# Chlumsky/msdfgen

Hardware: AMD Instinct MI355X
Metric: MSDF glyphs/sec (64x64, fp32) (higher is better)
Workload: dtype f64

## Files before the change

### msdfgen_amd/csrc/msdf_ec_fast.hpp

```cpp
#pragma once

#include "msdf_ec.hpp"

namespace msdfhip {

enum { EC_DEFER = 0x80 };

enum { EC_V_ERROR = 1,
       EC_V_CHECK = 2,
       EC_V_COND = 4,
       EC_V_HELD = 8 };
enum { EC_ORDER_EAGER = 0, EC_ORDER_LAZY = 1, EC_ORDER_LAZY_HELD = 2 };

MSDF_HD bool ecHasBasePass(const EcParams &p) { return p.distanceCheck == EC_DO_NOT_CHECK || (p.distanceCheck == EC_CHECK_AT_EDGE && p.mode != EC_MODE_EDGE_ONLY); }
MSDF_HD bool ecHasShapePass(const EcParams &p) { return p.distanceCheck == EC_ALWAYS_CHECK || p.distanceCheck == EC_CHECK_AT_EDGE; }
MSDF_HD bool ecLazyProtect(const EcParams &p) { return p.mode == EC_MODE_EDGE_PRIORITY && p.distanceCheck == EC_CHECK_AT_EDGE; }

struct FastCtx {
    double span;
    bool p1;
    bool pShape;
    bool basePass, shapePass;
    int order;
};

MSDF_HD int rangeTest2(const FastCtx &c, double at, double bt, double xt, float am, float bm, float xm) {
    const bool inversion = (am > .5f && bm > .5f && xm <= .5f) || (am < .5f && bm < .5f && xm >= .5f);
    const bool outside = medianf(am, bm, xm) != xm;
    const bool candBase = c.basePass && (inversion || (!c.p1 && outside));
    const bool candShape = c.shapePass && (inversion || (!c.pShape && outside));
    const bool candCond = c.order != EC_ORDER_EAGER && !inversion && outside;
    if (!(candBase || candShape || candCond))
        return 0;
    const double axSpan = (xt-at)*c.span, bxSpan = (bt-xt)*c.span;
    const int f = (xm >= am-axSpan && xm <= am+axSpan && xm >= bm-bxSpan && xm <= bm+bxSpan) ? 1 : 3;
    return (candBase ? f : 0)|(candShape ? f<<2 : 0)|(candCond && f == 3 ? 16 : 0);
}

MSDF_HD int judge(int flags) {
    const int cond = (flags&16) ? EC_V_COND : 0;
    if (flags&2)
        return EC_V_ERROR|cond;
    const int fs = (flags>>2)&3;
    if (fs&1)
        return ((fs&2) ? EC_V_ERROR : EC_V_CHECK)|cond;
    return cond;
}

MSDF_HD bool quadraticMayHaveRootInRange(double a, double b, double c) {
    if (a == 0 || fabs(b) > 1e12*fabs(a))
        return true;
    const double lo = .005, hi = .995;
    const double mag = fabs(a)+fabs(b)+fabs(c);
    const double eps = 1e-9*mag;
    const double flo = (a*lo+b)*lo+c, fhi = (a*hi+b)*hi+c;
    if (!(flo > eps && fhi > eps) && !(flo < -eps && fhi < -eps))
        return true;
    const double s = flo > 0 ? 1. : -1.;
    const double as = a*s, bs = b*s, cs = c*s;
    if (as <= 0)
        return false;
    if (!(-bs > 2*as*lo*(1-1e-9) && -bs < 2*as*hi*(1+1e-9)))
        return false;
    return !(4*as*cs-bs*bs > 1e-9*mag*mag);
}

MSDF_HD bool bernsteinMayHaveRoot(float dA, float dBC, float dD) {
    const float m = fmaxf(fmaxf(fabsf(dA), fabsf(dBC)), fabsf(dD));
    const float eps = 1e-5f*m;
    const float h = .5f*dBC;
    return !((dA > eps && h > eps && dD > eps) || (dA < -eps && h < -eps && dD < -eps));
}

MSDF_HD bool edgeBetweenTexelsChannelFast(const float *a, const float *b, int channel) {
    const double n = a[channel]-.5;
    const double d = a[channel]-b[channel];
    if (!((n > 0 && d > 0 && n < d) || (n < 0 && d < 0 && n > d)))
        return false;
    const double t = n/d;
    if (t > 0 && t < 1) {
        float c[3] = { mixf(a[0], b[0], t), mixf(a[1], b[1], t), mixf(a[2], b[2], t) };
        return medianf(c[0], c[1], c[2]) == c[channel];
    }
    return false;
}

MSDF_HD int edgeBetweenTexelsFast(const float *a, const float *b) {
    return 1*(int) edgeBetweenTexelsChannelFast(a, b, 0)+2*(int) edgeBetweenTexelsChannelFast(a, b, 1)+4*(int) edgeBetweenTexelsChannelFast(a, b, 2);
}

template <class Sink>
MSDF_HD int diagonalPairFast(const FastCtx &cx, float am, float dm, const float *a, const float *l, const float *q,
                             float dA, float dBC, float dD, float l0, float q0, float l1, float q1, Sink &sink) {
    const double qa = dD-dBC+dA, qb = dBC-dA-dA, qc = dA;
    if (!quadraticMayHaveRootInRange(qa, qb, qc))
        return 0;
    double t[2];
    const int solutions = solveQuadratic(t, qa, qb, qc);
    int verdict = 0;
    for (int i = 0; i < solutions; ++i) {
        if (t[i] > MSDF_ARTIFACT_T_EPSILON && t[i] < 1-MSDF_ARTIFACT_T_EPSILON) {
            const float xm = interpolatedMedianQuad(a, l, q, t[i]);
            int rangeFlags = rangeTest2(cx, 0, 1, t[i], am, dm, xm);
            const double tEx0 = -.5*l0/q0, tEx1 = -.5*l1/q1;
            if (tEx0 > 0 && tEx0 < 1) {
                double tEnd0 = 0, tEnd1 = 1;
                float em0 = am, em1 = dm;
                const float ex = interpolatedMedianQuad(a, l, q, tEx0);
                if (tEx0 > t[i])
                    tEnd1 = tEx0, em1 = ex;
                else
                    tEnd0 = tEx0, em0 = ex;
                rangeFlags |= rangeTest2(cx, tEnd0, tEnd1, t[i], em0, em1, xm);
            }
            if (tEx1 > 0 && tEx1 < 1) {
                double tEnd0 = 0, tEnd1 = 1;
                float em0 = am, em1 = dm;
                const float ex = interpolatedMedianQuad(a, l, q, tEx1);
                if (tEx1 > t[i])
                    tEnd1 = tEx1, em1 = ex;
                else
                    tEnd0 = tEx1, em0 = ex;
                rangeFlags |= rangeTest2(cx, tEnd0, tEnd1, t[i], em0, em1, xm);
            }
            const int v = judge(rangeFlags);
            verdict |= v;
            if (v&EC_V_CHECK) {
                const bool held = (verdict&EC_V_COND) != 0;
                if (held)
                    verdict |= EC_V_HELD;
                if (held == (cx.order == EC_ORDER_LAZY_HELD))
                    sink(t[i]);
            }
            if (verdict&EC_V_ERROR)
                return verdict;
        }
    }
    return verdict;
}

struct Neighbourhood {
    float v[3][3][3];
    float dev[3][3];
    unsigned valid;
};

MSDF_HD float ecTexelDeviation(const float *t) { return fabsf(medianf(t[0], t[1], t[2])-.5f); }

MSDF_HD void loadNeighbourhood(Neighbourhood &nb, const SdfView &sdf, int x, int yn) {
    nb.valid = 0;
    MSDF_UNROLL
    for (int dy = -1; dy <= 1; ++dy) {
        MSDF_UNROLL
        for (int dx = -1; dx <= 1; ++dx) {
            const int nx = x+dx, ny = yn+dy;
            const bool in = nx >= 0 && ny >= 0 && nx < sdf.w && ny < sdf.h;
            const float *t = sdf.native(in ? nx : x, in ? ny : yn);
            nb.v[dy+1][dx+1][0] = t[0], nb.v[dy+1][dx+1][1] = t[1], nb.v[dy+1][dx+1][2] = t[2];
            nb.dev[dy+1][dx+1] = ecTexelDeviation(t);
            if (in)
                nb.valid |= 1u<<((dy+1)*3+(dx+1));
        }
    }
}

template <class Emit>
MSDF_HD void texelProtectPairs(const Neighbourhood &nb, const EcParams &p, Emit &emit) {
    const float sdev = nb.dev[1][1];
    MSDF_UNROLL
    for (int dy = -1; dy <= 1; ++dy) {
        MSDF_UNROLL
        for (int dx = -1; dx <= 1; ++dx) {
            if (!dx && !dy)
                continue;
            if (!(nb.valid&(1u<<((dy+1)*3+(dx+1)))))
                continue;
            const float radius = dy == 0 ? p.radiusH : dx == 0 ? p.radiusV : p.radiusD;
            const float odev = nb.dev[dy+1][dx+1];
            const bool selfIsA = dy > 0 || (dy == 0 && dx > 0);
            const float sum = selfIsA ? sdev+odev : odev+sdev;
            if (sum < radius)
                emit((dy+1)*3+(dx+1));
        }
    }
}

MSDF_HD bool evaluateProtectPair(const float *self, const float *other, int m) {
    const int dy = m/3-1, dx = m%3-1;
    const bool selfIsA = dy > 0 || (dy == 0 && dx > 0);
    const int mask = selfIsA ? edgeBetweenTexelsFast(self, other) : edgeBetweenTexelsFast(other, self);
    return extremeChannelInMask(self, medianf(self[0], self[1], self[2]), mask);
}

MSDF_HD bool protectedByEdgesNb(const Neighbourhood &nb, const EcParams &p) {
    struct Items {
        unsigned char m[8];
        int n;
        MSDF_HD void operator()(int mm) { m[n++] = (unsigned char) mm; }
    } items;
    items.n = 0;
    texelProtectPairs(nb, p, items);
    for (int i = 0; i < items.n; ++i)
        if (evaluateProtectPair(nb.v[1][1], nb.v[items.m[i]/3][items.m[i]%3], items.m[i]))
            return true;
    return false;
}

MSDF_HD int ecNeighbourDx(int k) { return k < 4 ? (k == 0 ? -1 : k == 2 ? 1 : 0) : ((k&1) ? 1 : -1); }
MSDF_HD int ecNeighbourDy(int k) { return k < 4 ? (k == 1 ? -1 : k == 3 ? 1 : 0) : ((k&2) ? 1 : -1); }

template <class Emit>
MSDF_HD void texelCandidatePairs(const Neighbourhood &nb, Emit &emit) {
    const float *c = nb.v[1][1];
    const float cdev = nb.dev[1][1];
    MSDF_UNROLL
    for (int k = 0; k < 4; ++k) {
        const int dx = k == 0 ? -1 : k == 2 ? 1 : 0, dy = k == 1 ? -1 : k == 3 ? 1 : 0;
        if (!(nb.valid&(1u<<((dy+1)*3+(dx+1)))))
            continue;
        const float *b = nb.v[dy+1][dx+1];
        if (!(cdev >= nb.dev[dy+1][dx+1]))
            continue;
        MSDF_UNROLL
        for (int j = 0; j < 3; ++j) {
            const int i0 = j, i1 = j == 2 ? 0 : j+1;
            const float dA = c[i1]-c[i0], dB = b[i1]-b[i0];
            if ((dA > 0 && dB < 0) || (dA < 0 && dB > 0))
                emit(k, j);
        }
    }
    MSDF_UNROLL
    for (int k = 4; k < 8; ++k) {
        const int dx = (k&1) ? 1 : -1, dy = (k&2) ? 1 : -1;
        if (!(nb.valid&(1u<<((dy+1)*3+(dx+1)))))
            continue;
        const float *d = nb.v[dy+1][dx+1];
        if (!(cdev >= nb.dev[dy+1][dx+1]))
            continue;
        const float *b = nb.v[1][dx+1], *cc = nb.v[dy+1][1];
        MSDF_UNROLL
        for (int j = 0; j < 3; ++j) {
            const int i0 = j, i1 = j == 2 ? 0 : j+1;
            const float dA = c[i1]-c[i0], dBC = b[i1]-b[i0]+cc[i1]-cc[i0], dD = d[i1]-d[i0];
            if (dA == 0 && dBC == 0 && dD == 0)
                continue;
            if (bernsteinMayHaveRoot(dA, dBC, dD))
                emit(k, j);
        }
    }
}

MSDF_HD float pick3(const float *v, int i) { return i == 0 ? v[0] : i == 1 ? v[1] : v[2]; }

template <class Sink>
MSDF_HD int evaluatePair(const float *c, const float *n, const float *hb, const float *vc, const EcParams &p, bool p1, int flip, int k, int j, Sink &sink,
                         int order = EC_ORDER_EAGER) {
    FastCtx cx;
    cx.basePass = ecHasBasePass(p);
    cx.shapePass = ecHasShapePass(p);
    cx.order = order;
    cx.p1 = order != EC_ORDER_EAGER || p1;
    cx.pShape = (p.distanceCheck == EC_CHECK_AT_EDGE) ? true : cx.p1;
    const int dx = ecNeighbourDx(k), dy = ecNeighbourDy(k);
    const int i0 = j, i1 = j == 2 ? 0 : j+1;
    const float cm = medianf(c[0], c[1], c[2]), nm = medianf(n[0], n[1], n[2]);
    if (k < 4) {
        if (order == EC_ORDER_LAZY_HELD)
            return 0;
        cx.span = dy == 0 ? p.hSpan : p.vSpan;
        const float dA = pick3(c, i1)-pick3(c, i0), dB = pick3(n, i1)-pick3(n, i0);
        const double t = (double) dA/(dA-dB);
        if (t > MSDF_ARTIFACT_T_EPSILON && t < 1-MSDF_ARTIFACT_T_EPSILON) {
            const float xm = interpolatedMedianLin(c, n, t);
            const int v = judge(rangeTest2(cx, 0, 1, t, cm, nm, xm));
            if (v&EC_V_CHECK)
                sink(t, dx, flip ? -dy : dy);
            return v;
        }
        return 0;
    }
    cx.span = p.dSpan;
    const float *a = c, *b = hb, *cc = vc, *d = n;
    const float abc[3] = { a[0]-b[0]-cc[0], a[1]-b[1]-cc[1], a[2]-b[2]-cc[2] };
    const float l[3] = { -a[0]-abc[0], -a[1]-abc[1], -a[2]-abc[2] };
    const float q[3] = { d[0]+abc[0], d[1]+abc[1], d[2]+abc[2] };
    const float a3[3] = { a[0], a[1], a[2] };
    struct DirSink {
        Sink &sink;
        int dx, dy;
        MSDF_HD void operator()(double t) { sink(t, dx, dy); }
    } dirSink = { sink, dx, flip ? -dy : dy };
    const float dA = pick3(a, i1)-pick3(a, i0), dBC = pick3(b, i1)-pick3(b, i0)+pick3(cc, i1)-pick3(cc, i0), dD = pick3(d, i1)-pick3(d, i0);
    return diagonalPairFast(cx, cm, nm, a3, l, q, dA, dBC, dD, pick3(l, i0), pick3(q, i0), pick3(l, i1), pick3(q, i1), dirSink);
}

template <class Sink>
MSDF_HD int texelFindFast(const Neighbourhood &nb, const EcParams &p, bool p1, int flip, Sink &sink, int order = EC_ORDER_EAGER) {
    struct Items {
        unsigned char k[24], j[24];
        int n;
        MSDF_HD void operator()(int kk, int jj) { k[n] = (unsigned char) kk, j[n] = (unsigned char) jj; ++n; }
    } items;
    items.n = 0;
    texelCandidatePairs(nb, items);
    int verdict = 0;
    for (int i = 0; i < items.n; ++i) {
        const int k = items.k[i], dx = ecNeighbourDx(k), dy = ecNeighbourDy(k);
        verdict |= evaluatePair(nb.v[1][1], nb.v[dy+1][dx+1], nb.v[1][dx+1], nb.v[dy+1][1], p, p1, flip, k, items.j[i], sink, order);
    }
    return verdict;
}

MSDF_HD bool protectedByCornerList(const int *corners, int nCorners, int x, int ys) {
    for (int i = 0; i < nCorners; ++i) {
        const int l = corners[2*i], b = corners[2*i+1];
        if ((x == l || x == l+1) && (ys == b || ys == b+1))
            return true;
    }
    return false;
}

MSDF_HD bool ecNeedsProtection(int verdict) { return ((verdict&EC_V_COND) && !(verdict&EC_V_ERROR)) || (verdict&EC_V_HELD); }

template <class Sink>
MSDF_HD int ecTexelFast(const SdfView &sdf, const EcParams &p, const int *corners, int nCorners, int x, int yn, Sink &sink, bool allowLazy = true) {
    const int ys = sdf.flip ? sdf.h-1-yn : yn;
    Neighbourhood nb;
    loadNeighbourhood(nb, sdf, x, yn);
    int st = 0, verdict;
    if (allowLazy && ecLazyProtect(p)) {
        verdict = texelFindFast(nb, p, true, sdf.flip, sink, EC_ORDER_LAZY);
        if (ecNeedsProtection(verdict)) {
            if (!(protectedByCornerList(corners, nCorners, x, ys) || protectedByEdgesNb(nb, p)))
                verdict |= EC_V_ERROR;
            else if (verdict&EC_V_HELD)
                texelFindFast(nb, p, true, sdf.flip, sink, EC_ORDER_LAZY_HELD);
        }
    } else {
        if (p.mode == EC_MODE_EDGE_PRIORITY) {
            if (protectedByCornerList(corners, nCorners, x, ys) || protectedByEdgesNb(nb, p))
                st |= EC_PROTECTED;
        } else if (p.mode == EC_MODE_EDGE_ONLY)
            st |= EC_PROTECTED;
        verdict = texelFindFast(nb, p, (st&EC_PROTECTED) != 0, sdf.flip, sink);
    }
    if (ecHasBasePass(p) && p.distanceCheck == EC_CHECK_AT_EDGE)
        st |= EC_PROTECTED;
    if (verdict&EC_V_ERROR)
        st |= EC_ERROR;
    else if (verdict&EC_V_CHECK)
        st |= EC_DEFER;
    return st;
}

template <class Query>
MSDF_HD bool ecEvaluateCandidate(const SdfView &sdf, const EcParams &p, int x, int ys, double t, int dx, int dy, const Query &query) {
    const float *msd = sdf.shape(x, ys);
    const V2 tVector = t*mk(dx, dy);
    float oldMSD[3], newMSD[3];
    interpolate3(oldMSD, sdf, mk(x+.5, ys+.5)+tVector);
    const double aWeight = (1-fabs(tVector.x))*(1-fabs(tVector.y));
    const float aPSD = medianf(msd[0], msd[1], msd[2]);
    newMSD[0] = (float) (oldMSD[0]+aWeight*(aPSD-msd[0]));
    newMSD[1] = (float) (oldMSD[1]+aWeight*(aPSD-msd[1]));
    newMSD[2] = (float) (oldMSD[2]+aWeight*(aPSD-msd[2]));
    const float oldPSD = medianf(oldMSD[0], oldMSD[1], oldMSD[2]);
    const float newPSD = medianf(newMSD[0], newMSD[1], newMSD[2]);
    const V2 q = unproject(p.t, mk(x+.5, ys+.5))+mk(tVector.x*p.texelX, tVector.y*p.texelY);
    const float refPSD = mapDistance(p.t, query(q));
    return p.minImproveRatio*fabsf(newPSD-refPSD) < (double) fabsf(oldPSD-refPSD);
}

}
```

### msdfgen_amd/csrc/msdf_kernels.hpp

```cpp
#pragma once

#include <hip/hip_runtime.h>
#include "msdf_device.hpp"
#include "msdf_prep.hpp"
#include "msdf_ec.hpp"
#include "msdf_ec_fast.hpp"
#include "msdf_cull.hpp"
#include "msdf_scanline.hpp"
#include "msdf_shapeprep.hpp"
#include "msdf_frame.hpp"
#include "../../include/msdfgen_hip.h"

namespace msdfhip {

#ifndef MSDF_DISTANCE_WAVES_PER_SIMD
#define MSDF_DISTANCE_WAVES_PER_SIMD 4
#endif
constexpr int TILE = 8;
constexpr int WAVE = 64;
constexpr int REC_DOUBLES = sizeof(EdgeRec)/sizeof(double);

struct BatchView {
    int nGlyphs;
    const int32_t *glyphContourOffsets;
// ... 781 lines not shown
    mutable unsigned long long cached;
    int cacheCap;
#if defined(MSDF_PROFILE_QUERY)
    mutable unsigned long long prof[16];
#endif
    MSDF_HD int begin(int c) const { return coff[c]-coff[0]; }
    MSDF_HD int end(int c) const { return coff[c+1]-coff[0]; }
};
#if defined(MSDF_PROFILE_QUERY)
__device__ inline unsigned long long qNow() {
#if MSDF_PROFILE_QUERY >= 2
    asm volatile("s_waitcnt vmcnt(0) lgkmcnt(0)" ::: "memory");
#endif
    return __builtin_readcyclecounter();
}
__device__ inline void profAdd(const EdgesCooperative &edges, int i, unsigned long long dt) { edges.prof[i] += dt; }
__device__ inline unsigned long long profNow(const EdgesCooperative &) { return qNow(); }
__device__ unsigned long long gQueryDetail[16];
#endif

__device__ inline void selAddContour(Selector<2> &sel, const EdgeRec *rec, const EdgesCooperative &edges, int c, V2 o) {
    if (edges.slots) {
        if (c == 0) {
#if defined(MSDF_PROFILE_QUERY)
            const unsigned long long qa = qNow();
#endif
            for (int base = 0; base < edges.nE; base += WAVE) {
                const int i = base+edges.lane;
                if (i < edges.nE) {
                    Selector<2> mine;
                    selInit(mine);
                    const EdgeRegs r = loadEdgeRegs(rec+i, i);
                    selAddEdge(mine, r, i, o);
                    edges.slots[i] = mine.c[0];
                }
            }
            waveSync();
#if defined(MSDF_PROFILE_QUERY)
            const unsigned long long qb = qNow();
            edges.prof[0] += qb-qa;
#endif
            for (int cc = edges.lane; cc < edges.C; cc += WAVE) {
                PB acc;
                pbInit(acc);
                const int e = edges.end(cc);
                for (int i = edges.begin(cc); i < e; ++i) {
                    const PBSlot one = edges.slots[i];
                    pbMerge(acc, one);
                }
                edges.merged[cc] = acc;
            }
            waveSync();
#if defined(MSDF_PROFILE_QUERY)
            edges.prof[1] += qNow()-qb;
#endif
        }
        const PBSlot whole = edges.merged[c];
        pbMerge(sel.c[0], whole);
        return;
    }
    const bool cacheable = c < 64 && c < edges.cacheCap;
    if (cacheable && ((edges.cached>>c)&1ull)) {
        const PBSlot whole = edges.merged[c];
        pbMerge(sel.c[0], whole);
        return;
    }
    PB contour;
    pbInit(contour);
    const int e = edges.end(c);
    for (int base = edges.begin(c); base < e; base += WAVE) {
        Selector<2> mine;
        selInit(mine);
        const int i = base+edges.lane;
        if (i < e) {
            const EdgeRegs r = loadEdgeRegs(rec+i, i);
            selAddEdge(mine, r, i, o);
        }
        PB &m = mine.c[0];
        MSDF_UNROLL
        for (int off = 1; off < WAVE; off <<= 1) {
            PB other;
            other.td = __shfl_down(m.td, off), other.tdot = __shfl_down(m.tdot, off), other.perp = __shfl_down(m.perp, off);
            other.neg = __shfl_down(m.neg, off), other.pos = __shfl_down(m.pos, off);
            if (edges.lane+off < WAVE)
                pbMerge(m, other);
        }
        PB all;
        all.td = __shfl(m.td, 0), all.tdot = __shfl(m.tdot, 0), all.perp = __shfl(m.perp, 0), all.neg = __shfl(m.neg, 0), all.pos = __shfl(m.pos, 0);
        pbMerge(contour, all);
    }
    pbMerge(sel.c[0], contour);
    if (cacheable) {
        edges.merged[c] = contour;
        edges.cached |= 1ull<<c;
        waveSync();
    }
}

template <bool OVERLAP, class Wind = const int8_t *>
struct PsdfQueryCooperative {
    const EdgeRec *rec;
    const int32_t *coff;
    Wind windings;
    int C, lane;
    double *res;
    PBSlot *slots, *merged;
    int cacheCap = 0;
    __device__ double operator()(V2 q) const {
        double out[1];
        EdgesCooperative edges;
        edges.coff = coff, edges.lane = lane, edges.slots = slots, edges.merged = merged, edges.nE = coff[C]-coff[0], edges.C = C;
        edges.cached = 0, edges.cacheCap = slots ? 0 : cacheCap;
#if defined(MSDF_PROFILE_QUERY)
        for (int i = 0; i < 16; ++i)
            edges.prof[i] = 0;
        const unsigned long long qq0 = qNow();
#endif
        if (slots)
            waveSync();
        if (OVERLAP)
            shapeDistanceOverlap<2>(rec, edges, windings, C, q, res, 1, out);
        else
            shapeDistanceSimple<2>(rec, edges, C, q, out);
#if defined(MSDF_PROFILE_QUERY)
        if (lane == 0) {
            atomicAdd(&gQueryDetail[0], 1ull), atomicAdd(&gQueryDetail[1], qNow()-qq0);
            atomicAdd(&gQueryDetail[2], edges.prof[0]), atomicAdd(&gQueryDetail[3], edges.prof[1]), atomicAdd(&gQueryDetail[4], edges.prof[8]);
            atomicAdd(&gQueryDetail[5], edges.prof[9]), atomicAdd(&gQueryDetail[6], edges.prof[10]), atomicAdd(&gQueryDetail[7], edges.prof[11]);
            atomicAdd(&gQueryDetail[8], (unsigned long long) C), atomicAdd(&gQueryDetail[9], (unsigned long long) (slots ? 1 : 0));
        }
#endif
        return out[0];
    }
};

struct EcCandidate {
    unsigned texel;
    int dir;
    double t;
};
static_assert(sizeof(EcCandidate) == 16, "EcCandidate layout");

MSDF_HD size_t ecHeaderRecords(int nGlyphs) { return ((size_t) (nGlyphs+1)*sizeof(unsigned)+sizeof(EcCandidate)-1)/sizeof(EcCandidate); }
MSDF_HD unsigned ecSegment(size_t texelsPerGlyph) { return (unsigned) (texelsPerGlyph/8 > 64 ? (texelsPerGlyph/8+63)/64*64 : 64); }

struct CandidateSink {
    unsigned *header;
    EcCandidate *segment;
    unsigned seg, texel;
    int g;
    __device__ void operator()(double t, int dx, int dy) {
        const unsigned slot = atomicAdd(&header[1+g], 1u);
        if (slot < seg) {
            EcCandidate c;
            c.texel = texel, c.dir = (dx+1)|((dy+1)<<2), c.t = t;
            segment[slot] = c;
        } else
            header[0] = 1u;
    }
};

MSDF_HD size_t stencilIndex(size_t texel, int yn, int width, int height, int stencilYDown) {
    return stencilYDown ? texel+(size_t) (height-1-2*yn)*width : texel;
}

struct EcGlyphParams {
    double hSpan, vSpan, dSpan, texelX, texelY;
    float radiusH, radiusV, radiusD;
    int cornerBegin, nCorners;
    int pad;
};
static_assert(sizeof(EcGlyphParams) == 64, "EcGlyphParams layout");

__device__ __forceinline__ void ecParamsBody(EcGlyphParams *out, const BatchView &batch, const MsdfHipGlyph *glyphs, const MsdfHipConfig &cfg, unsigned *candidateHeader,
                                             int *corners, int *sizes, const int g, const int lane) {
    if (candidateHeader && lane == 0) {
        candidateHeader[1+g] = 0;
        if (g == 0)
            candidateHeader[0] = 0;
    }
    EcParams p;
    p.t = loadXform(glyphs[g]);
    p.minDeviationRatio = cfg.min_deviation_ratio;
    p.minImproveRatio = cfg.min_improve_ratio;
    ecDerive(p);
    const int c0 = batch.glyphContourOffsets[g], C = batch.glyphContourOffsets[g+1]-c0;
    const int e0 = batch.contourOffsets[c0], nE = batch.contourOffsets[c0+C]-e0;
    int nCorners = 0;
    if (cfg.ec_mode == EC_MODE_EDGE_PRIORITY && corners) {
        const EdgeRec *rec = batch.recs+e0;
        for (int base = 0; base < nE; base += WAVE) {
            const int e = base+lane;
            const bool corner = e < nE && (rec[e].flags&REC_CORNER);
            const unsigned long long mask = __ballot(corner);
            if (corner) {
                const V2 pp = project(p.t, ld(rec[e].p0));
                const int slot = e0+nCorners+__popcll(mask&((1ull<<lane)-1ull));
                corners[2*slot] = (int) floor(pp.x-.5);
                corners[2*slot+1] = (int) floor(pp.y-.5);
            }
            nCorners += __popcll(mask);
        }
    }
    if (lane == 0) {
        EcGlyphParams o;
        o.hSpan = p.hSpan, o.vSpan = p.vSpan, o.dSpan = p.dSpan, o.texelX = p.texelX, o.texelY = p.texelY;
        o.radiusH = p.radiusH, o.radiusV = p.radiusV, o.radiusD = p.radiusD, o.cornerBegin = e0, o.nCorners = nCorners, o.pad = 0;
        out[g] = o;
        if (sizes)
            sizes[2*g] = nE, sizes[2*g+1] = C;
    }
}
__global__ void __launch_bounds__(WAVE)
k_ec_params(EcGlyphParams *out, BatchView batch, const MsdfHipGlyph *glyphs, MsdfHipConfig cfg, unsigned *candidateHeader, int *corners, int *sizes) {
    ecParamsBody(out, batch, glyphs, cfg, candidateHeader, corners, sizes, (int) blockIdx.x, (int) threadIdx.x);
}

#ifndef MSDF_EC_FAST_WAVES_PER_SIMD
#define MSDF_EC_FAST_WAVES_PER_SIMD 7
#endif
enum { EC_HALO = TILE+2, EC_QUEUE_CAP = WAVE*24, EC_PROTECT_QUEUE_CAP = WAVE*8 };
__host__ __device__ inline size_t ecFastLdsBytes(int maxEdges, int n) {
    return (size_t) EC_HALO*EC_HALO*n*sizeof(float)+(WAVE+4)*sizeof(int)
           +(EC_QUEUE_CAP+EC_PROTECT_QUEUE_CAP)*sizeof(unsigned short);
}

__device__ __forceinline__ bool ecTileCornerTexel(const int *list, int nCorners, int tx, int ty, int height, int flip, int lane) {
    const int lxT = lane&(TILE-1), lyT = lane>>3;
    const int xT = tx*TILE+lxT, ysT = flip ? height-1-(ty*TILE+lyT) : ty*TILE+lyT;
    const int x0 = tx*TILE, x1 = tx*TILE+TILE-1;
    const int ya = flip ? height-1-(ty*TILE+TILE-1) : ty*TILE, yb = flip ? height-1-ty*TILE : ty*TILE+TILE-1;
    bool cornerTexel = false;
    for (int base = 0; base < nCorners; base += WAVE) {
        const int k = base+lane;
        int l = 0, b = 0;
        bool near = false;
        if (k < nCorners) {
            l = list[2*k], b = list[2*k+1];
            near = l+1 >= x0 && l <= x1 && b+1 >= ya && b <= yb;
        }
        for (unsigned long long mask = __ballot(near); mask; mask &= mask-1) {
            const int src = __ffsll((long long) mask)-1;
            const int cl = __builtin_amdgcn_readlane(l, src), cb = __builtin_amdgcn_readlane(b, src);
            cornerTexel = cornerTexel || ((xT == cl || xT == cl+1) && (ysT == cb || ysT == cb+1));
        }
    }
    return cornerTexel;
}

template <int N>
__device__ __forceinline__ void ecRunProtectQueue(const float *halo, const unsigned short *protectQueue, int nProtect, int *verdictLds, int lane) {
    for (int base = 0; base < nProtect; base += WAVE) {
        const int it = base+lane;
        if (it >= nProtect)
            continue;
        const unsigned item = protectQueue[it];
        const int s = item&63, m = item>>6;
        const int sx = s&(TILE-1), sy = s>>3;
        const float *self = halo+((sy+1)*EC_HALO+sx+1)*N, *other = halo+((sy+m/3)*EC_HALO+sx+m%3)*N;
        if (evaluateProtectPair(self, other, m))
            atomicOr(&verdictLds[s], 0x100);
    }
}

struct EcPushProtect {
    unsigned short *queue;
    int *count;
    int lane;
    __device__ void operator()(int m) { queue[atomicAdd(count, 1)] = (unsigned short) (lane|m<<6); }
};

template <int N, int ORDER = -1>
__device__ __forceinline__ void ecFastBody(const BatchView &batch, const MsdfHipGlyph *glyphs, int width, int height, int tilesX, int tilesPerGlyph,
          const float *src, float *out, uint8_t *stencilOut, const MsdfHipConfig &cfg, const EcGlyphParams *glyphParams, EcCandidate *cands, unsigned seg,
          int maxEdges, const int *corners, const unsigned blockId, int *smemFast, const int sinkSlots = 0, const int sinkSlot = 0) {
    const GlyphWork wk = decodeItem(blockId, batch.nGlyphs, tilesPerGlyph);
    if (!wk.valid)
        return;
    float *halo = reinterpret_cast<float *>(smemFast);
    int *verdictLds = reinterpret_cast<int *>(halo+EC_HALO*EC_HALO*N);
    int *itemCount = verdictLds+WAVE;
    unsigned short *queue = reinterpret_cast<unsigned short *>(itemCount+4);
    unsigned short *protectQueue = queue+EC_QUEUE_CAP;
    float *devLds = reinterpret_cast<float *>(queue+EC_QUEUE_CAP)-EC_HALO*EC_HALO;
    static_assert((EC_QUEUE_CAP*sizeof(unsigned short))%sizeof(float) == 0 && EC_QUEUE_CAP*sizeof(unsigned short) >= EC_HALO*EC_HALO*sizeof(float), "devLds overlays the queue's tail");
    const int lane = threadIdx.x;
    const MsdfHipGlyph gd = glyphs[wk.g];
    EcParams p;
    p.t = loadXform(gd);
    p.minDeviationRatio = cfg.min_deviation_ratio;
    p.minImproveRatio = cfg.min_improve_ratio;
    p.mode = cfg.ec_mode, p.distanceCheck = cfg.ec_distance_check, p.overlap = cfg.overlap_support, p.stageLimit = 0;
    const EcGlyphParams gp = glyphParams[wk.g];
    p.hSpan = gp.hSpan, p.vSpan = gp.vSpan, p.dSpan = gp.dSpan, p.texelX = gp.texelX, p.texelY = gp.texelY;
    p.radiusH = gp.radiusH, p.radiusV = gp.radiusV, p.radiusD = gp.radiusD;
    const int tx = wk.tile%tilesX, ty = wk.tile/tilesX;

    const bool lazy = ORDER < 0 ? ecLazyProtect(p) : ORDER != 0;
    bool cornerTexel = false;
    if (p.mode == EC_MODE_EDGE_PRIORITY && !lazy)
        cornerTexel = ecTileCornerTexel(corners+2*(size_t) gp.cornerBegin, gp.nCorners, tx, ty, height, gd.flip, lane);

    const float *field = src+(size_t) wk.g*height*width*N;
    for (int idx = lane; idx < EC_HALO*EC_HALO; idx += WAVE) {
        const int hx = tx*TILE+idx%EC_HALO-1, hy = ty*TILE+idx/EC_HALO-1;
        if (hx >= 0 && hy >= 0 && hx < width && hy < height) {
            const float *t = field+((size_t) hy*width+hx)*N;
            float tv[N];
            for (int ch = 0; ch < N; ++ch)
                tv[ch] = t[ch], halo[idx*N+ch] = tv[ch];
            devLds[idx] = ecTexelDeviation(tv);
        }
    }
    if (lane < 2)
        itemCount[lane] = 0;
    waveSync();

    const int lx = lane&(TILE-1), ly = lane>>3;
    const int x = tx*TILE+lx, yn = ty*TILE+ly;
    const bool inside = x < width && yn < height;
    int st = 0;
    const bool classify = inside;
    Neighbourhood nb;
    nb.valid = 0;
    if (classify) {
        MSDF_UNROLL
        for (int dy = -1; dy <= 1; ++dy) {
            MSDF_UNROLL
            for (int dx = -1; dx <= 1; ++dx) {
                const int nx = x+dx, ny = yn+dy;
                const bool in = nx >= 0 && ny >= 0 && nx < width && ny < height;
                const float *t = halo+((ly+1+(in ? dy : 0))*EC_HALO+lx+1+(in ? dx : 0))*N;
                nb.v[dy+1][dx+1][0] = t[0], nb.v[dy+1][dx+1][1] = t[1], nb.v[dy+1][dx+1][2] = t[2];
                nb.dev[dy+1][dx+1] = devLds[(ly+1+(in ? dy : 0))*EC_HALO+lx+1+(in ? dx : 0)];
                if (in)
                    nb.valid |= 1u<<((dy+1)*3+(dx+1));
            }
        }
    }
    waveSync();
    if (classify) {
        if (p.mode == EC_MODE_EDGE_PRIORITY && !lazy) {
            if (cornerTexel)
                st |= EC_PROTECTED;
            if (!(st&EC_PROTECTED)) {
                EcPushProtect pushProtect = { protectQueue, itemCount+1, lane };
                texelProtectPairs(nb, p, pushProtect);
            }
        } else if (p.mode == EC_MODE_EDGE_ONLY)
            st |= EC_PROTECTED;
        struct Push {
            unsigned short *queue;
            int *count;
            int lane;
            __device__ void operator()(int k, int j) { queue[atomicAdd(count, 1)] = (unsigned short) (lane|k<<6|j<<9); }
        } push = { queue, itemCount, lane };
        texelCandidatePairs(nb, push);
    }
    verdictLds[lane] = (st&EC_PROTECTED) ? 0x100 : 0;
    waveSync();

    if (!lazy) {
        ecRunProtectQueue<N>(halo, protectQueue, itemCount[1], verdictLds, lane);
        waveSync();
    }

    const int nItems = itemCount[0];
    const auto runItems = [&](const int order) {
        for (int base = 0; base < nItems; base += WAVE) {
            const int it = base+lane;
            if (it >= nItems)
                continue;
            const unsigned item = queue[it];
            const int s = item&63, k = (item>>6)&7, jp = item>>9;
            const int word = verdictLds[s];
            if (order == EC_ORDER_LAZY_HELD && (word&(0x100|EC_V_HELD)) != (0x100|EC_V_HELD))
                continue;
            const int sx = s&(TILE-1), sy = s>>3;
            const int dx = ecNeighbourDx(k), dy = ecNeighbourDy(k);
            const float *c = halo+((sy+1)*EC_HALO+sx+1)*N, *n = halo+((sy+1+dy)*EC_HALO+sx+1+dx)*N;
            const float *hb = halo+((sy+1)*EC_HALO+sx+1+dx)*N, *vc = halo+((sy+1+dy)*EC_HALO+sx+1)*N;
            CandidateSink sink;
            sink.header = reinterpret_cast<unsigned *>(cands);
            sink.segment = sinkSlots > 0 ? cands+ecHeaderRecords(sinkSlots)+(size_t) sinkSlot*seg : cands+ecHeaderRecords(batch.nGlyphs)+(size_t) wk.g*seg;
            sink.seg = seg, sink.g = sinkSlots > 0 ? sinkSlot : wk.g;
            sink.texel = (unsigned) (((size_t) wk.g*height+ty*TILE+sy)*width+tx*TILE+sx);
            const int v = evaluatePair(c, n, hb, vc, p, (word&0x100) != 0, gd.flip, k, jp, sink, order);
            if (v && order != EC_ORDER_LAZY_HELD)
                atomicOr(&verdictLds[s], v);
        }
    };
    runItems(lazy ? EC_ORDER_LAZY : EC_ORDER_EAGER);
    waveSync();

    const bool need = lazy && inside && ecNeedsProtection(verdictLds[lane]);
    if (__ballot(need)) {
        __asm__ volatile("" ::: "memory");
        const EcGlyphParams gl = glyphParams[wk.g];
        EcParams pr = p;
        pr.radiusH = gl.radiusH, pr.radiusV = gl.radiusV, pr.radiusD = gl.radiusD;
        cornerTexel = ecTileCornerTexel(corners+2*(size_t) gl.cornerBegin, gl.nCorners, tx, ty, height, gd.flip, lane);
        if (need) {
            if (cornerTexel)
                verdictLds[lane] |= 0x100;
            else {
                Neighbourhood nd;
                nd.valid = 0;
                MSDF_UNROLL
                for (int dy = -1; dy <= 1; ++dy) {
                    MSDF_UNROLL
                    for (int dx = -1; dx <= 1; ++dx) {
                        const int nx = x+dx, ny = yn+dy;
                        const bool in = nx >= 0 && ny >= 0 && nx < width && ny < height;
                        nd.dev[dy+1][dx+1] = ecTexelDeviation(halo+((ly+1+(in ? dy : 0))*EC_HALO+lx+1+(in ? dx : 0))*N);
                        if (in)
                            nd.valid |= 1u<<((dy+1)*3+(dx+1));
                    }
                }
                EcPushProtect pushProtect = { protectQueue, itemCount+1, lane };
                texelProtectPairs(nd, pr, pushProtect);
            }
        }
        waveSync();
        ecRunProtectQueue<N>(halo, protectQueue, itemCount[1], verdictLds, lane);
        waveSync();
        bool revisit = false;
        if (need) {
            const int word = verdictLds[lane];
            if (!(word&0x100))
                verdictLds[lane] = word|EC_V_ERROR;
            revisit = (word&0x100) && (word&EC_V_HELD);
        }
        if (__ballot(revisit)) {
            waveSync();
            runItems(EC_ORDER_LAZY_HELD);
        }
    }

    if (!inside)
        return;
    const int verdict = verdictLds[lane];
    if ((verdict&0x100) || (ecHasBasePass(p) && p.distanceCheck == EC_CHECK_AT_EDGE))
        st |= EC_PROTECTED;
    if (verdict&EC_V_ERROR)
        st |= EC_ERROR;
    const size_t texel = ((size_t) wk.g*height+yn)*width+x;
    const float *in = halo+((ly+1)*EC_HALO+lx+1)*N;
    float v[N];
    for (int i = 0; i < N; ++i)
        v[i] = in[i];
    if (st&EC_ERROR) {
        const float m = medianf(v[0], v[1], v[2]);
        v[0] = m, v[1] = m, v[2] = m;
    }
    float *px = out+gd.out_offset+(ptrdiff_t) gd.row_stride*yn+(ptrdiff_t) N*x;
    for (int i = 0; i < N; ++i)
        px[i] = v[i];
    if (stencilOut)
        stencilOut[stencilIndex(texel, yn, width, height, cfg.stencil_y_down)] = (uint8_t) st;
}
template <int N, bool LAZY>
__global__ void __launch_bounds__(WAVE, MSDF_EC_FAST_WAVES_PER_SIMD)
k_ec_fast(BatchView batch, const MsdfHipGlyph *glyphs, int width, int height, int tilesX, int tilesPerGlyph,
          const float *src, float *out, uint8_t *stencilOut, MsdfHipConfig cfg, const EcGlyphParams *glyphParams, EcCandidate *cands, unsigned seg,
          int maxEdges, const int *corners) {
    extern __shared__ int smemFast[];
    ecFastBody<N, LAZY ? 1 : 0>(batch, glyphs, width, height, tilesX, tilesPerGlyph, src, out, stencilOut, cfg, glyphParams, cands, seg, maxEdges, corners, blockIdx.x, smemFast);
}

struct EcQueryPolicy { int lpcMaxContours, lpcEdgeCost, lpcMaxEdges, lpcMinCount, wideMaxEdges; float wideLoad, wideMeanCount; int gridSteps; };
MSDF_HD int ecQueryGridSlices(unsigned count, int nE, int C, EcQueryPolicy q) {
    if (q.gridSteps <= 0 || C > q.lpcMaxContours || count == 0)
        return 0;
    int J = 1;
    while (J < (int) count && J < WAVE)
        J <<= 1;
    int S = WAVE/J, need = 1;
    while (need*q.gridSteps < nE && need < WAVE)
        need <<= 1;
    if (need > S)
        S = need;
    return S >= 2 && S <= WAVE/2 ? S : 0;
}
MSDF_HD bool ecQueryLanePerCandidate(unsigned count, int nE, int C, EcQueryPolicy q) {
    if (C > q.lpcMaxContours)
        return false;
    if ((nE > q.lpcMaxEdges && (int) count < q.lpcMinCount))
        return false;
    const long long coop = (long long) count*(340ll*((nE+WAVE-1)/WAVE)+10ll*nE+1000ll);
    const long long lpc = (long long) ((count+WAVE-1)/WAVE)*((long long) q.lpcEdgeCost*nE+1000ll);
    return lpc < coop;
}
MSDF_HD int ecQueryItems(unsigned count, unsigned seg, int nE, int C, EcQueryPolicy lpcMaxContours) {
    if (count > seg)
        return 0;
    const int S = ecQueryGridSlices(count, nE, C, lpcMaxContours);
    if (S)
        return (int) ((count+WAVE/S-1)/(WAVE/S));
    return ecQueryLanePerCandidate(count, nE, C, lpcMaxContours) ? (int) ((count+WAVE-1)/WAVE) : (int) count;
}
MSDF_HD bool ecQueryListedFirst(unsigned count, int nE, int C, EcQueryPolicy q) {
    return ecQueryGridSlices(count, nE, C, q) != 0 || ecQueryLanePerCandidate(count, nE, C, q) || (q.gridSteps > 0 && nE > WAVE);
}

MSDF_HD size_t ecQueuesAt(int nGlyphs) { return 2*((size_t) nGlyphs+1)+2+2*(size_t) nGlyphs; }
MSDF_HD size_t ecOffsetInts(int nGlyphs) { return ecQueuesAt(nGlyphs)+8*16; }
MSDF_HD size_t ecSizesAt(int nGlyphs) { return 2*((size_t) nGlyphs+1)+2; }

__global__ void __launch_bounds__(1024)
k_ec_scan(int nGlyphs, const unsigned *__restrict__ header, unsigned seg, int *__restrict__ offsets, EcQueryPolicy lpcMaxContours, const int *__restrict__ order) {
    __shared__ int waveTotals[2][16];
    __shared__ float waveLoad[16], waveCount[16];
    enum { PER = 8 };
    const int t = threadIdx.x, lane = t&(WAVE-1), wave = t/WAVE;
    const int *sizes = offsets+ecSizesAt(nGlyphs);
    float mine = 0, mineCount = 0;
    for (int base = 0; base < nGlyphs; base += 1024*PER) {
        unsigned count[PER];
        int nE[PER];
        MSDF_UNROLL
        for (int k = 0; k < PER; ++k) {
            const int p = base+t*PER+k;
            const int g = p < nGlyphs ? (order ? order[p] : p) : -1;
            count[k] = g >= 0 ? header[1+g] : 0u, nE[k] = g >= 0 ? sizes[2*g] : 0;
        }
        MSDF_UNROLL
        for (int k = 0; k < PER; ++k)
            if (count[k] <= seg)
                mine += (float) count[k]*(340.f*((nE[k]+WAVE-1)/WAVE)+10.f*nE[k]+1000.f), mineCount += (float) count[k];
    }
    for (int off = WAVE/2; off > 0; off >>= 1)
        mine += __shfl_down(mine, off), mineCount += __shfl_down(mineCount, off);
    if (lane == 0)
        waveLoad[wave] = mine, waveCount[wave] = mineCount;
    __syncthreads();
    float total = 0, totalCount = 0;
    for (int w = 0; w < 16; ++w)
        total += waveLoad[w], totalCount += waveCount[w];
    const bool dense = lpcMaxContours.wideMeanCount > 0 && totalCount >= lpcMaxContours.wideMeanCount*(float) nGlyphs;
    if ((total > lpcMaxContours.wideLoad || dense) && lpcMaxContours.wideMaxEdges > lpcMaxContours.lpcMaxEdges)
        lpcMaxContours.lpcMaxEdges = lpcMaxContours.wideMaxEdges;
    const bool gridOff = total > lpcMaxContours.wideLoad || dense || lpcMaxContours.gridSteps <= 0;
    if (gridOff)
        lpcMaxContours.gridSteps = 0;
    int *coop = offsets+nGlyphs+1;
    int carry[2] = { 0, 0 };
    for (int base = 0; base < nGlyphs; base += 1024*PER) {
        int items[PER];
        bool chunky[PER];
        int sum[2] = { 0, 0 };
        MSDF_UNROLL
        for (int k = 0; k < PER; ++k) {
            const int p = base+t*PER+k;
            const int g = p < nGlyphs ? (order ? order[p] : p) : -1;
            const unsigned count = g >= 0 ? header[1+g] : 0u;
            const int nE = g >= 0 ? sizes[2*g] : 0, C = g >= 0 ? sizes[2*g+1] : 0;
            chunky[k] = g >= 0 && ecQueryListedFirst(count, nE, C, lpcMaxContours);
            items[k] = g >= 0 ? ecQueryItems(count, seg, nE, C, lpcMaxContours) : 0;
            sum[chunky[k] ? 0 : 1] += items[k];
        }
        int incl[2] = { sum[0], sum[1] };
        for (int off = 1; off < WAVE; off <<= 1) {
            const int n0 = __shfl_up(incl[0], off), n1 = __shfl_up(incl[1], off);
            if (lane >= off)
                incl[0] += n0, incl[1] += n1;
        }
        if (lane == WAVE-1)
            waveTotals[0][wave] = incl[0], waveTotals[1][wave] = incl[1];
        __syncthreads();
        int before[2] = { 0, 0 }, all[2] = { 0, 0 };
        for (int w = 0; w < 16; ++w) {
            const int v0 = waveTotals[0][w], v1 = waveTotals[1][w];
            if (w < wave)
                before[0] += v0, before[1] += v1;
            all[0] += v0, all[1] += v1;
        }
        int at[2] = { carry[0]+before[0]+incl[0]-sum[0], carry[1]+before[1]+incl[1]-sum[1] };
        MSDF_UNROLL
        for (int k = 0; k < PER; ++k) {
            const int p = base+t*PER+k;
            if (p < nGlyphs) {
                offsets[p] = at[0], coop[p] = at[1];
                at[chunky[k] ? 0 : 1] += items[k];
            }
        }
        carry[0] += all[0], carry[1] += all[1];
        __syncthreads();
    }
    if (t == 1023) {
        offsets[nGlyphs] = carry[0];
        coop[nGlyphs] = carry[1];
        coop[nGlyphs+1] = 0;
        for (int q = 0; q < 8; ++q)
            offsets[ecQueuesAt(nGlyphs)+16*q] = 0;
        coop[nGlyphs+2] = lpcMaxContours.lpcMaxEdges|(gridOff ? 1<<30 : 0);
    }
}

#ifndef MSDF_EC_QUERY_WAVES_PER_SIMD
#define MSDF_EC_QUERY_WAVES_PER_SIMD 3
#endif
#if defined(MSDF_PROFILE_QUERY)
__device__ unsigned long long gQueryProfile[24];
#if MSDF_PROFILE_QUERY >= 2
#define MSDF_QSTAMP(x) asm volatile("s_waitcnt vmcnt(0) lgkmcnt(0)" ::: "memory"); const unsigned long long x = __builtin_readcyclecounter()
#else
#define MSDF_QSTAMP(x) const unsigned long long x = __builtin_readcyclecounter()
#endif
#endif
template <int N, bool OVERLAP>
__global__ void __launch_bounds__(WAVE, MSDF_EC_QUERY_WAVES_PER_SIMD)
k_ec_query(int nGlyphs, const int32_t *__restrict__ glyphContourOffsets, const int32_t *__restrict__ contourOffsets, const EdgeRec *__restrict__ recs,
           const int8_t *__restrict__ windings, const MsdfHipGlyph *__restrict__ glyphs, int width, int height, const float *__restrict__ src, float *__restrict__ out,
           uint8_t *__restrict__ stencilOut, MsdfHipConfig cfg, const EcGlyphParams *__restrict__ glyphParams, const EcCandidate *__restrict__ cands, unsigned seg,
           const int *__restrict__ offsets, int *__restrict__ counter, int itemsPerTicket, int slotCap, int slotOffset, EcQueryPolicy lpcMaxContours,
           unsigned *__restrict__ overflowOut, const int *__restrict__ order, int queryFlags) {
    if (overflowOut && blockIdx.x == 0 && threadIdx.x == 0)
        *overflowOut = reinterpret_cast<const unsigned *>(cands)[0];
    BatchView batch;
    batch.nGlyphs = nGlyphs, batch.glyphContourOffsets = glyphContourOffsets, batch.contourOffsets = contourOffsets, batch.recs = recs, batch.windings = windings;
    extern __shared__ double smemLds[];
    PBSlot *slotBuf = reinterpret_cast<PBSlot *>(smemLds+slotOffset);
    const unsigned *header = reinterpret_cast<const unsigned *>(cands);
    const size_t texelsPerGlyph = (size_t) width*height;
    const int chunks = offsets[batch.nGlyphs], coopItems = offsets[2*batch.nGlyphs+1];
    const int tickets = chunks+(coopItems+itemsPerTicket-1)/itemsPerTicket;
    lpcMaxContours.lpcMaxEdges = offsets[2*batch.nGlyphs+3]&((1<<30)-1);
    if (offsets[2*batch.nGlyphs+3]&(1<<30))
        lpcMaxContours.gridSteps = 0;
#if defined(MSDF_PROFILE_QUERY)
    MSDF_QSTAMP(qStart);
    unsigned long long qAcc[8] = { 0, 0, 0, 0, 0, 0, 0, 0 }, qItems[4] = { 0, 0, 0, 0 }, qLongest = 0, qLastWork = 0, qLongestWho = 0;
#endif
    const int dealt = (queryFlags&1) ? (int) gridDim.x : 0;
    for (int round = 0;; ++round) {
#if defined(MSDF_PROFILE_QUERY)
        MSDF_QSTAMP(q0);
#endif
        int ticket = 0;
        if (dealt && (queryFlags&4) && round > 0) {
            const int q = (int) blockIdx.x&7;
            if (threadIdx.x == 0)
                ticket = atomicAdd(counter+(ecQueuesAt(batch.nGlyphs)-(2*(size_t) batch.nGlyphs+2))+16*q, 1);
            ticket = dealt+__builtin_amdgcn_readfirstlane(ticket)*8+q;
            if (ticket >= tickets)
                break;
        } else if (dealt) {
            if ((long long) round*dealt >= tickets)
                break;
            ticket = (round&1) ? (round+1)*dealt-1-(int) blockIdx.x : round*dealt+(int) blockIdx.x;
            if (ticket >= tickets)
                continue;
        } else {
            if (threadIdx.x == 0)
                ticket = atomicAdd(counter, 1);
            ticket = __builtin_amdgcn_readfirstlane(ticket);
            if (ticket >= tickets)
                break;
        }
#if defined(MSDF_PROFILE_QUERY)
        MSDF_QSTAMP(q1);
        qAcc[0] += q1-q0;
#endif
        const int *part = ticket < chunks ? offsets : offsets+batch.nGlyphs+1;
        const int first = ticket < chunks ? ticket : (ticket-chunks)*itemsPerTicket;
        const int last = ticket < chunks ? first+1 : (first+itemsPerTicket < coopItems ? first+itemsPerTicket : coopItems);
        int lo = 0, hi = batch.nGlyphs-1;
        while (lo < hi) {
            const int mid = (lo+hi)>>1;
            if (part[mid+1] > first)
                hi = mid;
            else
                lo = mid+1;
        }
        int pos = lo;
        MSDF_NOUNROLL
        for (int i = first; i < last; ++i) {
#if defined(MSDF_PROFILE_QUERY)
        MSDF_QSTAMP(q2a);
#endif
        while (part[pos+1] <= i)
            ++pos;
        const int item = i-part[pos];
        const int g = order ? order[pos] : pos;
#if defined(MSDF_PROFILE_QUERY)
        MSDF_QSTAMP(q2);
        qAcc[1] += q2-(i == first ? q1 : q2a);
#endif
        const unsigned count = header[1+g];
        const EcCandidate *segment = cands+ecHeaderRecords(batch.nGlyphs)+(size_t) g*seg;
        const int c0 = batch.glyphContourOffsets[g], C = batch.glyphContourOffsets[g+1]-c0;
        const int32_t *coff = batch.contourOffsets+c0;
        const MsdfHipGlyph gd = glyphs[g];
        EcParams p;
        p.t = loadXform(gd);
        p.minDeviationRatio = cfg.min_deviation_ratio;
        p.minImproveRatio = cfg.min_improve_ratio;
        p.mode = cfg.ec_mode, p.distanceCheck = cfg.ec_distance_check, p.overlap = OVERLAP, p.stageLimit = 0;
        const EcGlyphParams gp = glyphParams[g];
        p.hSpan = gp.hSpan, p.vSpan = gp.vSpan, p.dSpan = gp.dSpan, p.texelX = gp.texelX, p.texelY = gp.texelY;
        p.radiusH = gp.radiusH, p.radiusV = gp.radiusV, p.radiusD = gp.radiusD;
        SdfView sdf;
        sdf.px = src+(size_t) g*texelsPerGlyph*N;
        sdf.w = width, sdf.h = height, sdf.N = N, sdf.flip = gd.flip;
        const int nE = coff[C]-coff[0];
        WindingMasks wind;
        wind.mem = batch.windings+c0;
        wind.pos = wind.neg = 0;
        if (OVERLAP) {
            const int w = (int) threadIdx.x < C ? (int) wind.mem[threadIdx.x] : 0;
            wind.pos = __ballot(w > 0), wind.neg = __ballot(w < 0);
        }
#if defined(MSDF_PROFILE_QUERY)
        MSDF_QSTAMP(q3);
        qAcc[2] += q3-q2;
        unsigned long long q4 = q3;
        const bool qChunk = ecQueryListedFirst(count, nE, C, lpcMaxContours);
#endif
        const int gridS = ecQueryGridSlices(count, nE, C, lpcMaxContours);
        if (gridS) {
            PsdfQueryGrid<OVERLAP, WindingMasks> query;
            query.rec = batch.recs+coff[0], query.coff = coff, query.windings = wind, query.C = C, query.res = smemLds+threadIdx.x;
            query.S = gridS, query.slice = (int) threadIdx.x&(gridS-1);
            const unsigned k = (unsigned) item*(unsigned) (WAVE/gridS)+threadIdx.x/(unsigned) gridS;
            if (k < count) {
                const EcCandidate cand = segment[k];
                const size_t texel = cand.texel;
                const int rem = (int) (texel-(size_t) g*texelsPerGlyph);
                const int yn = rem/width, x = rem%width;
                const int ys = gd.flip ? height-1-yn : yn;
                const bool artifact = ecEvaluateCandidate(sdf, p, x, ys, cand.t, (cand.dir&3)-1, ((cand.dir>>2)&3)-1, query);
                if (artifact && query.slice == 0) {
                    const float *in = sdf.native(x, yn);
                    const float m = medianf(in[0], in[1], in[2]);
                    float *px = out+gd.out_offset+(ptrdiff_t) gd.row_stride*yn+(ptrdiff_t) N*x;
                    px[0] = m, px[1] = m, px[2] = m;
                    if (stencilOut)
                        stencilOut[stencilIndex(texel, yn, width, height, cfg.stencil_y_down)] |= (uint8_t) EC_ERROR;
                }
            }
        } else if (ecQueryLanePerCandidate(count, nE, C, lpcMaxContours)) {
            PsdfQuery<OVERLAP, WindingMasks, EdgesAllBatched> query;
            query.rec = batch.recs+coff[0], query.coff = coff, query.windings = wind, query.C = C, query.res = smemLds+threadIdx.x;
            const unsigned k = (unsigned) item*WAVE+threadIdx.x;
            if (k < count) {
                const EcCandidate cand = segment[k];
                const size_t texel = cand.texel;
                const int rem = (int) (texel-(size_t) g*texelsPerGlyph);
                const int yn = rem/width, x = rem%width;
                const int ys = gd.flip ? height-1-yn : yn;
                const bool artifact = ecEvaluateCandidate(sdf, p, x, ys, cand.t, (cand.dir&3)-1, ((cand.dir>>2)&3)-1, query);
                if (artifact) {
                    const float *in = sdf.native(x, yn);
                    const float m = medianf(in[0], in[1], in[2]);
                    float *px = out+gd.out_offset+(ptrdiff_t) gd.row_stride*yn+(ptrdiff_t) N*x;
                    px[0] = m, px[1] = m, px[2] = m;
                    if (stencilOut)
                        stencilOut[stencilIndex(texel, yn, width, height, cfg.stencil_y_down)] |= (uint8_t) EC_ERROR;
                }
            }
        } else {
            const EcCandidate cand = segment[item];
// ... 574 lines not shown
```

Before: 1.828 million.

## Skip error-correction classification for tiles with quiet channel ordering

Adds a per-tile 'quiet' test: while loading the halo, each lane votes (via wave ballots) on whether the channel orderings across all halo texels are consistent and bounded. If every channel pair keeps a consistent order, the tile cannot contain clashing texels, so it writes the texels through unchanged with a fixed stencil byte and skips the neighbourhood classification and item passes. The halo load becomes two fixed rounds with clamped addresses, so every lane reads a texel even when it lies out of bounds. This adds a few ballots per tile, and it relies on the ordering test being a sound proof that no error correction is needed.

Measured after the change: 1.844 million, median of 6. About the same (+0.9%).

```diff
diff --git a/msdfgen_amd/csrc/msdf_ec_fast.hpp b/msdfgen_amd/csrc/msdf_ec_fast.hpp
--- a/msdfgen_amd/csrc/msdf_ec_fast.hpp
+++ b/msdfgen_amd/csrc/msdf_ec_fast.hpp
@@ -70,6 +70,47 @@
     const float eps = 1e-5f*m;
     const float h = .5f*dBC;
     return !((dA > eps && h > eps && dD > eps) || (dA < -eps && h < -eps && dD < -eps));
+}
+
+#define EC_ORDER_T 0.00390625f
+#define EC_ORDER_V 64.f
+
+template <class Vote>
+MSDF_HD void ecOrderVotes(const float *t, Vote &vote) {
+    const bool unbounded = !(fabsf(t[0]) <= EC_ORDER_V && fabsf(t[1]) <= EC_ORDER_V && fabsf(t[2]) <= EC_ORDER_V);
+    MSDF_UNROLL
+    for (int j = 0; j < 3; ++j) {
+        const int i0 = j, i1 = j == 2 ? 0 : j+1;
+        const float d = t[i1]-t[i0];
+        vote(3*j, !(d > EC_ORDER_T));
+        vote(3*j+1, !(d < -EC_ORDER_T));
+        vote(3*j+2, !(d == 0));
+    }
+    vote(9, unbounded);
+}
+template <class Mask>
+MSDF_HD bool ecOrderVotesQuiet(const Mask *bad) {
+    return (!(bad[0]|bad[9]) || !(bad[1]|bad[9]) || !bad[2]) && (!(bad[3]|bad[9]) || !(bad[4]|bad[9]) || !bad[5]) && (!(bad[6]|bad[9]) || !(bad[7]|bad[9]) || !bad[8]);
+}
+
+MSDF_HD int ecQuietStencilByte(const EcParams &p) {
+    if (ecHasBasePass(p) && p.distanceCheck == EC_CHECK_AT_EDGE)
+        return EC_PROTECTED;
+    if (p.mode == EC_MODE_EDGE_PRIORITY)
+        return -1;
+    return p.mode == EC_MODE_EDGE_ONLY ? EC_PROTECTED : 0;
+}
+
+MSDF_HD bool ecTileQuiet(const SdfView &sdf, int tx, int ty, int tile) {
+    struct Vote {
+        bool bad[10];
+        MSDF_HD void operator()(int i, bool b) { bad[i] = bad[i] || b; }
+    } vote = { { false, false, false, false, false, false, false, false, false, false } };
+    for (int hy = ty*tile-1; hy <= ty*tile+tile; ++hy)
+        for (int hx = tx*tile-1; hx <= tx*tile+tile; ++hx)
+            if (hx >= 0 && hy >= 0 && hx < sdf.w && hy < sdf.h)
+                ecOrderVotes(sdf.native(hx, hy), vote);
+    return ecOrderVotesQuiet(vote.bad);
 }
 
 MSDF_HD bool edgeBetweenTexelsChannelFast(const float *a, const float *b, int channel) {
diff --git a/msdfgen_amd/csrc/msdf_kernels.hpp b/msdfgen_amd/csrc/msdf_kernels.hpp
--- a/msdfgen_amd/csrc/msdf_kernels.hpp
+++ b/msdfgen_amd/csrc/msdf_kernels.hpp
@@ -1107,13 +1107,24 @@
         cornerTexel = ecTileCornerTexel(corners+2*(size_t) gp.cornerBegin, gp.nCorners, tx, ty, height, gd.flip, lane);
 
     const float *field = src+(size_t) wk.g*height*width*N;
-    for (int idx = lane; idx < EC_HALO*EC_HALO; idx += WAVE) {
-        const int hx = tx*TILE+idx%EC_HALO-1, hy = ty*TILE+idx/EC_HALO-1;
-        if (hx >= 0 && hy >= 0 && hx < width && hy < height) {
-            const float *t = field+((size_t) hy*width+hx)*N;
-            float tv[N];
+    struct OrderVote {
+        unsigned long long bad[10];
+        __device__ void operator()(int i, bool b) { bad[i] |= __ballot(b); }
+    } orderVote = { { 0, 0, 0, 0, 0, 0, 0, 0, 0, 0 } };
+    MSDF_UNROLL
+    for (int round = 0; round < 2; ++round) {
+        const int idx = lane+round*WAVE, at = idx < EC_HALO*EC_HALO ? idx : EC_HALO*EC_HALO-1;
+        const int hx = tx*TILE+at%EC_HALO-1, hy = ty*TILE+at/EC_HALO-1;
+        const bool in = idx < EC_HALO*EC_HALO && hx >= 0 && hy >= 0 && hx < width && hy < height;
+        const int cx = hx < 0 ? 0 : hx < width ? hx : width-1, cy = hy < 0 ? 0 : hy < height ? hy : height-1;
+        const float *t = field+((size_t) cy*width+cx)*N;
+        float tv[N];
+        for (int ch = 0; ch < N; ++ch)
+            tv[ch] = t[ch];
+        ecOrderVotes(tv, orderVote);
+        if (in) {
             for (int ch = 0; ch < N; ++ch)
-                tv[ch] = t[ch], halo[idx*N+ch] = tv[ch];
+                halo[idx*N+ch] = tv[ch];
             devLds[idx] = ecTexelDeviation(tv);
         }
     }
@@ -1124,6 +1135,32 @@
     const int lx = lane&(TILE-1), ly = lane>>3;
     const int x = tx*TILE+lx, yn = ty*TILE+ly;
     const bool inside = x < width && yn < height;
+    const auto writeTexel = [&](const int stencil, const bool error) {
+        const size_t texel = ((size_t) wk.g*height+yn)*width+x;
+        const float *in = halo+((ly+1)*EC_HALO+lx+1)*N;
+        float v[N];
+        for (int i = 0; i < N; ++i)
+            v[i] = in[i];
+        if (error) {
+            const float m = medianf(v[0], v[1], v[2]);
+            v[0] = m, v[1] = m, v[2] = m;
+        }
+        float *px = out+gd.out_offset+(ptrdiff_t) gd.row_stride*yn+(ptrdiff_t) N*x;
+        for (int i = 0; i < N; ++i)
+            px[i] = v[i];
+        if (stencilOut)
+            stencilOut[stencilIndex(texel, yn, width, height, cfg.stencil_y_down)] = (uint8_t) stencil;
+    };
+
+    {
+        const int quietByte = ORDER == 1 ? (int) EC_PROTECTED : ecQuietStencilByte(p);
+        if (ecOrderVotesQuiet(orderVote.bad) && (quietByte >= 0 || !stencilOut)) {
+            if (inside)
+                writeTexel(quietByte, false);
+            return;
+        }
+    }
+
     int st = 0;
     const bool classify = inside;
     Neighbourhood nb;
@@ -1249,20 +1286,7 @@
         st |= EC_PROTECTED;
     if (verdict&EC_V_ERROR)
         st |= EC_ERROR;
-    const size_t texel = ((size_t) wk.g*height+yn)*width+x;
-    const float *in = halo+((ly+1)*EC_HALO+lx+1)*N;
-    float v[N];
-    for (int i = 0; i < N; ++i)
-        v[i] = in[i];
-    if (st&EC_ERROR) {
-        const float m = medianf(v[0], v[1], v[2]);
-        v[0] = m, v[1] = m, v[2] = m;
-    }
-    float *px = out+gd.out_offset+(ptrdiff_t) gd.row_stride*yn+(ptrdiff_t) N*x;
-    for (int i = 0; i < N; ++i)
-        px[i] = v[i];
-    if (stencilOut)
-        stencilOut[stencilIndex(texel, yn, width, height, cfg.stencil_y_down)] = (uint8_t) st;
+    writeTexel(st, (st&EC_ERROR) != 0);
 }
 template <int N, bool LAZY>
 __global__ void __launch_bounds__(WAVE, MSDF_EC_FAST_WAVES_PER_SIMD)
```
